# Black-Phoenix/CUDA-SfM

Measured on AMD Instinct MI355X. Metric: RANSAC E-matrix hypotheses/sec (8-point, fused scoring), inlier-mask parity vs CPU oracle, higher is better.
Workload: dtype f32

## Files before the change

### cuda-sfm_amd/csrc/common.hpp

```cpp
#pragma once
#include <hip/hip_runtime.h>
#include <stdint.h>
#include <stddef.h>
#include <string>
#include <atomic>
#include <type_traits>
#include "../../include/sfm_amd.h"
#include "pair_state.hpp"
#include "job_order.hpp"
#if SFM_AB
#include "../../include/sfm_amd_ab.h"
#endif

#if SFM_AB
#define SFM_SW(p, i) ((p).reserved[i])
#else
#define SFM_SW(p, i) 0
#endif

namespace sfm {

void set_error(const char *fmt, ...);

#define SFM_HIP_TRY(expr)                                                                      \
// ... 221 lines not shown
    hipEvent_t cells_ev = nullptr;
    hipStream_t cells_stream = nullptr;
    uint32_t cells_cap = 0, cells_mask = 0, cells_epoch = 0;
    uint32_t cand_h0 = 0, cand_seed = 0;
    const int32_t *cand_indices = nullptr;
    int cand_sweeps = 0;
    bool cand_given = false;
    hipStream_t pipe_stream = nullptr;
    hipEvent_t pipe_final[2] = { nullptr, nullptr }, pipe_call = nullptr;
    uint64_t *pipe_keys = nullptr;
    unsigned long long pipe_step = 0;
    bool pipe_pending = false;
    bool holds_ctx_ref = false;
    sfm::PairState state;
    float h_Kinv[9] = {};
    int pose_mode = SFM_POSE_REFERENCE;
    float *d_rstate = nullptr;
    float *d_rpoints = nullptr;
    float *d_rreproj = nullptr;
    void *d_rwork = nullptr;
    float *d_vstate = nullptr;
    float *d_vreproj = nullptr;
    void *d_vwork = nullptr;
    void *d_vhyp = nullptr;
    int *d_vcounts = nullptr;
    size_t cap_vhyps = 0;
    uint32_t view_hyps = 0;
    void *d_awork = nullptr;
    void *d_lwork = nullptr;
    void *d_lhyp = nullptr;
    size_t cap_lhyps = 0;
    int last_kernel = 0, last_grid = 0, last_block = 0, last_lds = 0;
};

namespace sfm {

int match_db_rows(const sfm_ctx *ctx, int n2);
int match_records(sfm_ctx *ctx, sfm_sift_point *d_sift1, int n1, const sfm_sift_point *d_sift2, int n2, int *out_idx);
int pose_chain(sfm_pair *pair, int mode, float *d_record);

int lane_contexts(sfm_ctx *ctx, int n, sfm_ctx **out);
int start_lanes_after(sfm_ctx *ctx, sfm_ctx *const *lanes, int n, hipEvent_t event);

int launch_ransac_score(sfm_pair *pair, ShardSlot &slot, hipStream_t stream, const sfm_ransac_params &p, uint32_t h0, uint32_t count,
                        unsigned long long *key2 = nullptr, const float *d_E_given = nullptr, bool serial = true);
int launch_ransac_finalize(sfm_pair *pair, const sfm_ransac_params &p, const unsigned long long *d_key, uint32_t hyp_host, bool from_key,
                           hipStream_t stream = nullptr, bool rederive = false);
int launch_permutation_indices(sfm_ctx *ctx, int n, uint32_t seed, int32_t *d_indices);
bool prefilter_usable(const sfm_pair *pair, const sfm_ransac_params &p, uint32_t count);
int prefilter_pick_rule(sfm_pair *pair, const sfm_ransac_params &p, uint32_t count);
int launch_score_prefilter(sfm_pair *pair, ShardSlot &slot, hipStream_t stream, const sfm_ransac_params &p, uint32_t h0, uint32_t count, unsigned long long *key2);
bool prefilter_sums_counts(const sfm_pair *pair, const sfm_ransac_params &p, uint32_t count);
int launch_pf_prep(sfm_pair *pair, ShardSlot &slot, hipStream_t stream, const sfm_ransac_params &p, uint32_t count);
int prefilter_tile_points(const sfm_pair *pair, const sfm_ransac_params &p);
int launch_pf_cells(sfm_pair *pair, hipStream_t stream, bool want_sorted = false, int tile = 0);
#if SFM_AB
int launch_score_prefilter_r2(sfm_pair *pair, ShardSlot &slot, hipStream_t stream, const sfm_ransac_params &p, uint32_t h0, uint32_t count, unsigned long long *key2);
int launch_score_mfma(sfm_pair *pair, ShardSlot &slot, hipStream_t stream, const sfm_ransac_params &p, uint32_t h0, uint32_t count);
int launch_prefilter_probe(sfm_ctx *ctx, const float *d_E, float thr, float B, const float pt[4], int survive_all, float *d_out);
int launch_prefilter_band_probe(sfm_ctx *ctx, const float *d_E, float thr, float B, const float box[8], int b_safe, const float pt[4], int survive_all, float *d_out);
#endif
int launch_ransac_fused(sfm_pair *pair, ShardSlot &slot, hipStream_t stream, const sfm_ransac_params &p, uint32_t h0, uint32_t count);
int launch_finalize_block(sfm_pair *pair, const sfm_ransac_params &p, const unsigned long long *d_key, uint32_t hyp_host, bool from_key,
                          hipStream_t stream, bool rederive);

int launch_fill_xu(sfm_pair *pair, const sfm_sift_point *d_data);
int launch_set_points(sfm_pair *pair, const float *d_X0, const float *d_X1);
int launch_pose_candidates(sfm_pair *pair, int mode);
int launch_choose_pose(sfm_pair *pair, int mode);
int launch_triangulate(sfm_pair *pair, int mode);
int launch_points_to_vbo(sfm_pair *pair, float *d_positions, float *d_velocities, float scale);
int launch_pair_record(sfm_pair *pair, int mode, float *d_record);
int launch_pose_chain(sfm_pair *pair, float *d_record);

int launch_refine(sfm_pair *pair, const sfm_refine_params &p);
int launch_refine_pairs(sfm_ctx *ctx, sfm_pair *const *pairs, int num_pairs, const sfm_refine_params &p, const uint8_t *const *d_masks);
size_t refine_work_bytes(int cap_points);
int refine_state_words();
int refine_pose_offset();
int refine_report_offset();

int launch_register(sfm_pair *pair, const sfm_sift_point *d_sift, const sfm_register_params &p, const float *d_points, const uint8_t *d_valid);
int launch_register_views(sfm_ctx *ctx, sfm_pair *const *pairs, int num_pairs, const sfm_sift_point *const *d_sifts, const sfm_register_params &p,
                          const float *const *d_points, const uint8_t *const *d_valid);
size_t register_work_bytes(int cap_points);
size_t register_hyp_bytes(size_t num_hypotheses);
int register_state_words();
int register_pose_offset();
int register_report_offset();

struct ViewPointsInputs { const sfm_sift_point *sift; const float *points; const uint8_t *valid; const float *pose2, *pose3; int pose_rows; };
int launch_view_points(sfm_pair *pair, const ViewPointsInputs &in, const sfm_view_points_params &p, const sfm_view_points_out &out);
int launch_view_points_views(sfm_ctx *ctx, sfm_pair *const *pairs, int num_pairs, const ViewPointsInputs *in, const sfm_view_points_params &p,
                             const sfm_view_points_out *outs);

struct AdjustInputs { const sfm_sift_point *sift; const float *points; const uint8_t *flags, *used2; const float *pose2, *pose3; int pose_rows; };
int launch_adjust(sfm_pair *pair, const AdjustInputs &in, const sfm_adjust_params &p, const sfm_adjust_out &out);
int launch_adjust_views(sfm_ctx *ctx, sfm_pair *const *pairs, int num_pairs, const AdjustInputs *in, const sfm_adjust_params &p, const sfm_adjust_out *outs);
size_t adjust_work_bytes(int cap_points);

struct AlignInputs { const float *points_a; const uint8_t *valid_a; const float *points_b; const uint8_t *valid_b; const int32_t *index; };
int launch_align(sfm_pair *a, sfm_pair *b, const AlignInputs &in, const sfm_align_params &p, const sfm_align_out &out);
int launch_align_pairs(sfm_ctx *ctx, sfm_pair *const *as, sfm_pair *const *bs, int num_links, const AlignInputs *in, const sfm_align_params &p,
                       const sfm_align_out *outs);
int launch_align_index(sfm_ctx *ctx, const sfm_sift_point *d_sift, int n, float min_score, float max_ambiguity, int32_t *d_index);
size_t align_work_bytes(int cap_points);
// ... 57 lines not shown
```

### cuda-sfm_amd/csrc/prefilter_lds.hpp

```cpp
#pragma once
#include "prefilter_record.hpp"

namespace sfm {

constexpr int kPfTileMax = 1024;
constexpr int kPfWaves = 16;
constexpr int kPfRing = 128;

constexpr int kPfERow = 10;
constexpr int kPfPassRows = 32, kPfPairRows = 64;
constexpr int pf_wave_bytes(int rows) { return rows * kPfERow * 4 + rows * 4; }
template <int RULE> struct PfLds {
    static constexpr int kFragsPerBlock = RULE == kPfRuleG ? 3 : 2;
    static constexpr int kBlockBytes = kFragsPerBlock * 64 * 16;
    static constexpr int kFrag = 0;
    static constexpr int kTileMax = kPfTileMax;
    int staged, pts, ring, wave, next, lut, bytes;
    __host__ __device__ explicit PfLds(int tile, int ring_entries = kPfRing, int entry_bytes = 8, int rows = RULE == kPfRuleG ? kPfPassRows : kPfPairRows)
    {
        staged = (tile + 63) & ~63;
        pts = kFrag + (staged / 32) * kBlockBytes;
        ring = pts + staged * 16;
        ring = (ring + ring_entries * entry_bytes - 1) & ~(ring_entries * entry_bytes - 1);
        wave = ring + kPfWaves * ring_entries * entry_bytes;
        next = wave + kPfWaves * pf_wave_bytes(rows);
        lut = next + 16;
        bytes = lut + kPfRingLutBytes;
    }
};
static_assert(kPfRing * 8 == 1024, "ring slots are addressed with (offset & 1023) | base");

static inline int pf_tile_points(int ld, int tmax)
{
    const int ntiles = (ld + tmax - 1) / tmax;
    const int t = ((ld + ntiles - 1) / ntiles + 31) & ~31;
    return t < 32 ? 32 : t;
}

constexpr unsigned long long kPfSumCountsMin = 1ull << 21;
static inline bool pf_sums_counts_at(unsigned count, int ld, int tile)
{
    return (unsigned long long)count * (unsigned long long)((ld + tile - 1) / tile) >= kPfSumCountsMin;
}

constexpr unsigned long long kPfPairPassesMin = 1ull << 22;
static inline bool pf_pairs_passes_at(unsigned count, int ld, int tile)
{
    return (unsigned long long)count * (unsigned long long)((ld + tile - 1) / tile) >= kPfPairPassesMin;
}

}
```

### cuda-sfm_amd/csrc/ransac.hip

```cpp
#include "ransac_device.hpp"
#include "block_ops.hpp"
#include "prefilter_record.hpp"

namespace sfm {

__device__ __forceinline__ void reset_keys(unsigned long long *key, unsigned long long *key2)
{
    if (blockIdx.x == 0 && threadIdx.x == 0) {
        key[0] = 0ull; key[1] = 0ull;
        if (key2) *key2 = 0ull;
    }
}

template <int WPE>
__global__ __launch_bounds__(64, WPE)
void ransac_solve_lanes(const float *__restrict__ X0, const float *__restrict__ X1, int ld, int n,
                        const int32_t *__restrict__ indices, uint32_t seed, uint32_t h0, uint32_t count,
                        int sweeps, float *__restrict__ Ecand, unsigned long long *zero_key, unsigned long long *zero_key2,
                        int *__restrict__ zero_counts, uint32_t *__restrict__ zero_ticks, uint32_t nzero)
{
    reset_keys(zero_key, zero_key2);
    const uint32_t i = blockIdx.x * blockDim.x + threadIdx.x;
    if (zero_ticks) for (uint32_t w = i; w < nzero; w += gridDim.x * blockDim.x) zero_ticks[w] = 0u;
    if (i >= count) return;
// ... 288 lines not shown
    sfm_ctx *ctx = pair->ctx;
    const uint32_t fused_max = p.jacobi_sweeps > 0 ? 4096u : 1024u;
    int kernel = p.kernel == SFM_KERNEL_AUTO ? (count <= fused_max ? SFM_KERNEL_FUSED : SFM_KERNEL_SPLIT) : p.kernel;
    if (d_E_given && kernel == SFM_KERNEL_FUSED) kernel = SFM_KERNEL_SPLIT;
    const bool self_clearing = !d_E_given && count > 0 && (kernel == SFM_KERNEL_SPLIT || kernel == SFM_KERNEL_PREFILTER);
    if (!self_clearing) {
        if (!pair->state.key_clean) SFM_HIP_TRY(hipMemsetAsync(s.key, 0, 2 * sizeof(unsigned long long), stream));
        if (key2) SFM_HIP_TRY(hipMemsetAsync(key2, 0, sizeof(unsigned long long), stream));
    }
    pair->state.key_clean = false;
    pair->state.last_count = serial ? count : 0;
    pair->cand_given = serial && d_E_given != nullptr;
    if (serial) { pair->cand_h0 = h0; pair->cand_seed = p.seed; pair->cand_indices = p.d_indices; pair->cand_sweeps = p.jacobi_sweeps; }
    if (count == 0) return SFM_OK;
    int rc = ensure_hyp_capacity(s, stream, count);
    if (rc != SFM_OK) return rc;

#if SFM_AB
    if (kernel == SFM_KERNEL_MFMA && pair->n >= 65536) kernel = SFM_KERNEL_SPLIT;
#endif
    if (kernel == SFM_KERNEL_PREFILTER && !prefilter_usable(pair, p, 0x40000000u)) kernel = SFM_KERNEL_SPLIT;
    if (p.kernel == SFM_KERNEL_AUTO && kernel == SFM_KERNEL_SPLIT && prefilter_usable(pair, p, count) && SFM_SW(p, 3) != 1) kernel = SFM_KERNEL_PREFILTER;
    pair->last_kernel = kernel;
    if (kernel == SFM_KERNEL_FUSED) {
        rc = launch_ransac_fused(pair, s, stream, p, h0, count);
        if (rc == SFM_OK && key2) SFM_HIP_TRY(hipMemcpyAsync(key2, s.key, sizeof(unsigned long long), hipMemcpyDeviceToDevice, stream));
        return rc;
    }

    const int tile = pair->ld < kTileMax ? pair->ld : kTileMax;
    const int ntiles = (pair->ld + tile - 1) / tile;
    int wpb = 16;
    while (wpb > 4 && (count + wpb - 1) / wpb < (uint32_t)ctx->num_cus) wpb >>= 1;
    const int nh = (wpb == 16 && count >= 8192u) ? 2 : 1;
    const uint32_t nbatch = (count + wpb * nh - 1) / (wpb * nh);
    const bool grid2d = ntiles > 1 && kernel == SFM_KERNEL_SPLIT && wpb == 16 && SFM_SW(p, 1) != 1;
    const bool prefilter = kernel == SFM_KERNEL_PREFILTER;

    const bool timed = ctx->timing && ctx->tcount < sfm_ctx::kTimingSlots;
    hipEvent_t *tev = timed ? ctx->tev[ctx->tcount] : nullptr;
    if (timed) SFM_HIP_TRY(hipEventRecord(tev[0], stream));
    const bool pf_tickets = prefilter && (SFM_SW(p, 3) == 2 || SFM_SW(p, 3) == 17);
    const bool pf_r2 = prefilter && SFM_SW(p, 3) == 2;
    PfScales pf_sc = {};
    if (prefilter) (void)prefilter_scales(p.threshold, pf_sc);
    if (prefilter && !pf_r2) {
        const int pf_rule = prefilter_pick_rule(pair, p, count);
        const int rcc = launch_pf_cells(pair, stream, pf_rule == kPfRuleBandTile, prefilter_tile_points(pair, p));
        if (rcc != SFM_OK) return rcc;
    }
    const bool pf_sums = prefilter && !pf_r2 && !pf_tickets && prefilter_sums_counts(pair, p, count);
    int *zero_counts = (grid2d || pf_tickets || pf_sums) ? s.counts : nullptr;
    const float4 *pts4 = (pair->state.have_pts4 && SFM_SW(p, 0) != 4) ? pair->d_pts4 : nullptr;
    const uint32_t nzero = (!prefilter || pf_sums) ? 0u : (pf_tickets ? (count + (uint32_t)kPfGroup - 1u) / (uint32_t)kPfGroup : 2u * count);
    uint32_t *zero_ticks = (prefilter && !pf_sums) ? s.tick : nullptr;
    if (zero_ticks && d_E_given) {
        SFM_HIP_TRY(hipMemsetAsync(s.tick, 0, (size_t)nzero * sizeof(uint32_t), stream));
        zero_ticks = nullptr;
    }
    bool need_prep = prefilter && !pf_r2;
    if (d_E_given) {
        SFM_HIP_TRY(hipMemcpyAsync(s.Ecand, d_E_given, (size_t)count * 9 * sizeof(float), hipMemcpyDeviceToDevice, stream));
        if (zero_counts) SFM_HIP_TRY(hipMemsetAsync(s.counts, 0, (size_t)count * sizeof(int), stream));
    }
#if SFM_AB
    else if (p.reserved[0] == 1 || p.reserved[0] == 7) {
        auto kern = p.reserved[0] == 1 ? ransac_solve_lanes<1> : ransac_solve_lanes<3>;
        hipLaunchKernelGGL(kern, dim3((count + 63) / 64), dim3(64), 0, stream,
                           pair->d_X[0], pair->d_X[1], pair->ld, pair->n, p.d_indices, p.seed, h0, count,
                           p.jacobi_sweeps, s.Ecand, s.key, key2, zero_counts, zero_ticks, nzero);
    }
#endif
    else if (p.jacobi_sweeps <= 0 && (SFM_SW(p, 0) == 3 || (SFM_SW(p, 0) == 0 && (pts4 != nullptr || count <= kScalarSolveMax)))) {
        const bool fuse = need_prep && SFM_SW(p, 3) != 3;
        const bool tile_rec = !fuse || pair->pf_rule == kPfRuleBandTile;
        hipLaunchKernelGGL(tile_rec ? ransac_solve_lanes1_qr : ransac_solve_lanes1_qr_rec, dim3((count + 63) / 64), dim3(64), 0, stream,
                           pair->d_X[0], pair->d_X[1], pair->ld, pair->n, p.d_indices, p.seed, h0, count,
                           p.jacobi_sweeps, s.Ecand, s.key, key2, zero_counts, zero_ticks, nzero, pts4,
                           fuse ? reinterpret_cast<PfRecord *>(s.pf) : nullptr, p.threshold, pf_sc, pair->d_bound, pair->d_cells, pair->cells_mask,
                           pair->pf_rule);
        if (fuse) need_prep = false;
    }
    else if (p.jacobi_sweeps <= 0)
        hipLaunchKernelGGL(ransac_solve_lanes2<true>, dim3((count + 127) / 128), dim3(64), 0, stream,
                           pair->d_X[0], pair->d_X[1], pair->ld, pair->n, p.d_indices, p.seed, h0, count,
                           p.jacobi_sweeps, s.Ecand, s.key, key2, zero_counts, zero_ticks, nzero, pts4);
#if SFM_AB
    else if (p.reserved[0] == 2)
        hipLaunchKernelGGL(ransac_solve_lanes2<false>, dim3((count + 127) / 128), dim3(64), 0, stream,
                           pair->d_X[0], pair->d_X[1], pair->ld, pair->n, p.d_indices, p.seed, h0, count,
                           p.jacobi_sweeps, s.Ecand, s.key, key2, zero_counts, zero_ticks, nzero, pts4);
#endif
    else
        hipLaunchKernelGGL(ransac_solve_lanes<2>, dim3((count + 63) / 64), dim3(64), 0, stream,
                           pair->d_X[0], pair->d_X[1], pair->ld, pair->n, p.d_indices, p.seed, h0, count,
                           p.jacobi_sweeps, s.Ecand, s.key, key2, zero_counts, zero_ticks, nzero);
    SFM_HIP_TRY(hipGetLastError());
    if (need_prep) {
        const int rcp = launch_pf_prep(pair, s, stream, p, count);
        if (rcp != SFM_OK) return rcp;
    }
    if (timed) SFM_HIP_TRY(hipEventRecord(tev[1], stream));

    const bool uz = pair->state.unit_z;
    const size_t lds = (uz ? (size_t)2 * kUnitZSecond : (size_t)6 * tile * sizeof(float)) + 16 * sizeof(unsigned long long);
    int per_cu = (int)((160 * 1024) / lds);
    if (per_cu > 2048 / (wpb * 64)) per_cu = 2048 / (wpb * 64);
    if (per_cu < 1) per_cu = 1;
    const uint32_t resident = (uint32_t)ctx->num_cus * (uint32_t)per_cu;
    const uint32_t min_batches = SFM_SW(p, 2) > 0 ? (uint32_t)SFM_SW(p, 2) : 8u;
    uint32_t blocks = nbatch / min_batches;
    if (blocks > 16u * (uint32_t)ctx->num_cus) blocks = 16u * (uint32_t)ctx->num_cus;
    if (blocks < resident) blocks = resident;
    int grid = (int)(nbatch < blocks ? nbatch : blocks);
    if (grid2d) {
        grid = (int)((blocks + ntiles - 1) / ntiles);
        if ((uint32_t)grid > nbatch) grid = (int)nbatch;
    }
    if (prefilter) {
#if SFM_AB
        if (pf_r2) rc = launch_score_prefilter_r2(pair, s, stream, p, h0, count, key2);
        else
#endif
        rc = launch_score_prefilter(pair, s, stream, p, h0, count, key2);
        if (rc == SFM_OK && pf_sums) rc = launch_argmax_counts(s, stream, h0, count, key2);
    }
#if SFM_AB
    else if (kernel == SFM_KERNEL_MFMA) {
        rc = launch_score_mfma(pair, s, stream, p, h0, count);
        if (rc == SFM_OK && key2) SFM_HIP_TRY(hipMemcpyAsync(key2, s.key, sizeof(unsigned long long), hipMemcpyDeviceToDevice, stream));
    }
#endif
    else if (grid2d) {
        rc = uz ? (nh == 2 ? launch_score_t<16, true, 2, true>(pair, s, stream, h0, count, p.threshold, tile, ntiles, grid, lds, key2)
                           : launch_score_t<16, true, 1, true>(pair, s, stream, h0, count, p.threshold, tile, ntiles, grid, lds, key2))
                : (nh == 2 ? launch_score_t<16, false, 2, true>(pair, s, stream, h0, count, p.threshold, tile, ntiles, grid, lds, key2)
                           : launch_score_t<16, false, 1, true>(pair, s, stream, h0, count, p.threshold, tile, ntiles, grid, lds, key2));
    }
    else if (uz) switch (wpb) {
    case 16: rc = nh == 2 ? launch_score_t<16, true, 2>(pair, s, stream, h0, count, p.threshold, tile, ntiles, grid, lds, key2)
                          : launch_score_t<16, true>(pair, s, stream, h0, count, p.threshold, tile, ntiles, grid, lds, key2); break;
    case 8:  rc = launch_score_t<8, true>(pair, s, stream, h0, count, p.threshold, tile, ntiles, grid, lds, key2); break;
    default: rc = launch_score_t<4, true>(pair, s, stream, h0, count, p.threshold, tile, ntiles, grid, lds, key2); break;
    }
    else switch (wpb) {
    case 16: rc = nh == 2 ? launch_score_t<16, false, 2>(pair, s, stream, h0, count, p.threshold, tile, ntiles, grid, lds, key2)
                          : launch_score_t<16, false>(pair, s, stream, h0, count, p.threshold, tile, ntiles, grid, lds, key2); break;
    case 8:  rc = launch_score_t<8, false>(pair, s, stream, h0, count, p.threshold, tile, ntiles, grid, lds, key2); break;
    default: rc = launch_score_t<4, false>(pair, s, stream, h0, count, p.threshold, tile, ntiles, grid, lds, key2); break;
    }
    if (rc == SFM_OK && timed) {
        SFM_HIP_TRY(hipEventRecord(tev[2], stream));
        ctx->tcount++;
    }
    return rc;
}

int launch_ransac_finalize(sfm_pair *pair, const sfm_ransac_params &p, const unsigned long long *d_key,
                           uint32_t hyp_host, bool from_key, hipStream_t stream, bool rederive)
{
    sfm_ctx *ctx = pair->ctx;
    if (!stream) stream = ctx->stream;
    (void)ctx;
    if (pair->cand_given && !rederive) {
        set_error("finalize after sfm_ransac_score_candidates: the candidates were supplied by the caller, not derived from 8-tuples");
        return SFM_E_STATE;
    }
    return launch_finalize_block(pair, p, d_key, hyp_host, from_key, stream, rederive);
}

int launch_permutation_indices(sfm_ctx *ctx, int n, uint32_t seed, int32_t *d_indices)
{
    const int h = n / 8;
    if (h == 0) return SFM_OK;
    int32_t *perm = new int32_t[n];
    for (int i = 0; i < n; ++i) perm[i] = i;
    const uint32_t base = hash32(hash32(seed) ^ 0x51F15EEDu);
    for (int i = n - 1; i > 0; --i) {
// ... 12 lines not shown
```

### cuda-sfm_amd/csrc/ransac_prefilter.hip

```cpp
#include "ransac_device.hpp"
#include "block_ops.hpp"
#include "prefilter_math.hpp"
#include "prefilter_record.hpp"
#include "prefilter_lds.hpp"

namespace sfm {

typedef float f16v __attribute__((ext_vector_type(16)));


__device__ constexpr int kPfESlot[9] = { 2, 6, 1, 3, 5, 7, 0, 4, 8 };
__device__ __forceinline__ uint32_t shift_in_reject(uint32_t rejected, float nt, float G)
{
    return __builtin_amdgcn_alignbit(rejected, __float_as_uint(fmaf(-nt, nt, G)), 31);
}

__device__ __forceinline__ uint32_t scan16(const f16v &nt, const f16v &G)
{
    uint32_t rejected = 0u;
#pragma unroll
    for (int r = 0; r < 16; ++r) rejected = shift_in_reject(rejected, nt[r], G[r]);
    return rejected;
}

// ... 38 lines not shown
    const v2f ab1 = __builtin_elementwise_fma(e44, yv, __builtin_elementwise_fma(e31, xu, p2));
    const float a2 = fmaf(p2.y, yv.x, fmaf(p0.y, xu.x, e8));
    const float nn = fmaf(yv.y, ab1.x, fmaf(xu.y, ab0.x, a2));
    const float n2 = nn * nn;
    const v2f dd = __builtin_elementwise_fma(ab1, ab1, ab0 * ab0);
    const float da = dd.x, db = dd.y;
    const float m = n2 * (da + db);
    const float tp = (da * db) * band.thr;
    const uint32_t mb = __float_as_uint(m), tb = __float_as_uint(tp);
    const uint32_t gap = __usad(mb, tb, 0u);
    const bool undecided = (gap < kBandUlps) || (tb < band.lo_bits) || (tb > band.hi_bits);
    bool in = m < tp;
    if (undecided) {
        const float t1 = (da == 0.0f) ? 0.0f : n2 / da;
        const float t2 = (db == 0.0f) ? 0.0f : n2 / db;
        in = (t1 + t2) < band.thr;
    }
    return in;
}

template <int RULE>
__device__ __forceinline__ PfFrags load_point_frags(lds_ch8 *frag_lane, int pb)
{
    lds_ch8 *p = frag_lane + pb * (PfLds<RULE>::kBlockBytes / 16);
    if (RULE != kPfRuleG) return PfFrags{ p[0], p[64], h8{} };
    return PfFrags{ p[0], p[64], p[128] };
}

template <int RULE>
__device__ __forceinline__ void mfma_step(const PfFrags &a, const PfFrags &b, f16v &G, f16v &nt)
{
    const f16v z = {};
    nt = __builtin_amdgcn_mfma_f32_32x32x16_f16(a.n0, b.n0, z, 0, 0, 0);
    if (RULE == kPfRuleG) G = __builtin_amdgcn_mfma_f32_32x32x16_f16(a.t, b.t, z, 0, 0, 0);
    nt = __builtin_amdgcn_mfma_f32_32x32x16_f16(a.n1, b.n1, nt, 0, 0, 0);
}

#define PF_SCHED_STEP()                                                 \
    do {                                                                \
        if (RULE != kPfRuleG) {                                         \
            __builtin_amdgcn_sched_group_barrier(0x008, 1, 0);          \
            __builtin_amdgcn_sched_group_barrier(0x002, 8, 0);          \
            __builtin_amdgcn_sched_group_barrier(0x008, 1, 0);          \
            __builtin_amdgcn_sched_group_barrier(0x002, 8, 0);          \
        } else {                                                        \
            __builtin_amdgcn_sched_group_barrier(0x008, 1, 0);          \
            __builtin_amdgcn_sched_group_barrier(0x002, 11, 0);         \
            __builtin_amdgcn_sched_group_barrier(0x008, 1, 0);          \
            __builtin_amdgcn_sched_group_barrier(0x002, 11, 0);         \
            __builtin_amdgcn_sched_group_barrier(0x008, 1, 0);          \
            __builtin_amdgcn_sched_group_barrier(0x002, 11, 0);         \
        }                                                               \
    } while (0)

constexpr int kPfVarTickets = 1;
constexpr int kPfVarDrainLocal = 2;
constexpr int kPfVarClosedDecode = 4;
constexpr int kPfVarAnswerEpilogue = 8;
constexpr int kPfVarDrainK1 = 16, kPfVarDrainK7 = 32;
constexpr int kPfVarSinglePass = 64;
constexpr int kPfVarPairDrain = 128;

constexpr int pf_score_waves_per_simd(int var, int rule, int fl2, int pipe, int wide, int prio)
{
    if ((var == 0 || var == kPfVarPairDrain) && rule == kPfRuleBandTile && !fl2 && !pipe && !wide && !prio) return 4;
    return ((var & kPfVarTickets) == 0 && (rule == kPfRuleBandTile || rule == kPfRuleBandPack) && !fl2 && !pipe && !wide && !prio) ? 5 : 4;
}

template <int W, int VAR = 0, int RULE = kPfRuleBandTile, int FL2 = 0, int PIPE = 0, int WIDE = 0, int PRIO = 0>
__global__ __launch_bounds__(W * 64, pf_score_waves_per_simd(VAR, RULE, FL2, PIPE, WIDE, PRIO))
void ransac_score_prefilter(const float *__restrict__ X0, const float *__restrict__ X1, int ld, int n,
                            const float *__restrict__ Ecand, const PfRecord *__restrict__ recs, uint32_t h0, uint32_t count, float thr,
                            int dynamic, int tile,
                            int *__restrict__ counts, uint32_t *__restrict__ tick,
                            unsigned long long *best_key, unsigned long long *best_key2, unsigned long long *__restrict__ clk,
                            const unsigned long long *__restrict__ bound_word, const uint32_t *__restrict__ tile_boxes)
{
    extern __shared__ __attribute__((aligned(16))) unsigned char smem[];
    const int lane = threadIdx.x & 63;
    const int wave = __builtin_amdgcn_readfirstlane(threadIdx.x >> 6);
    const bool probe = clk && blockIdx.x == 0 && blockIdx.y == 0 && threadIdx.x == 0;
    unsigned long long c0 = 0, w0 = 0;
    if (clk && blockIdx.x == 0 && blockIdx.y == 0 && wave == 0) { c0 = clock64(); w0 = wall_clock64(); }
#if SFM_AB
    const uint32_t trace_blk = blockIdx.y * gridDim.x + blockIdx.x;
    unsigned long long *trace = (clk && trace_blk < (uint32_t)kTraceBlocks) ? clk + 8 + (size_t)trace_blk * kTraceWords : nullptr;
    if (trace && threadIdx.x == 0) {
        trace[0] = wall_clock64();
        trace[2] = ((unsigned long long)__builtin_amdgcn_s_getreg((20 << 0) | (0 << 6) | (31 << 11)) << 32) |
                   (unsigned long long)__builtin_amdgcn_s_getreg((4 << 0) | (0 << 6) | (31 << 11));
        trace[3] = ((unsigned long long)blockIdx.y << 32) | blockIdx.x;
    }
#define PF_PHASE(k) do { if (probe1) clk[k] = wall_clock64() - w0; } while (0)
#else
#define PF_PHASE(k) do { } while (0)
#endif
    const int half = lane >> 5, row = lane & 31;
    uint32_t npass = (count + (uint32_t)kPfGroup - 1u) / (uint32_t)kPfGroup;
    const uint32_t nstatic = gridDim.x * (uint32_t)W;
    using LT = PfLds<RULE>;
    constexpr bool kBand = RULE != kPfRuleG, kTile = RULE == kPfRuleBandTile, kPack = RULE == kPfRuleBandPack || kTile;
    static_assert(!(FL2 && kPack) && !((VAR & kPfVarTickets) && kPack), "the recorded variants were built on the v_alignbit scan");
    constexpr bool kTail9 = kPack && W == 16 && !FL2 && !PIPE && !WIDE && !PRIO && !(VAR & kPfVarTickets);
    static_assert(kTail9 || (VAR & ~kPfVarTickets) == 0, "the pass-tail switches belong to the product's two rules");
    static_assert(!(VAR & kPfVarSinglePass) || (kTile && VAR == kPfVarSinglePass), "single passes: the per-tile rule's summing instance");
    static_assert(!(VAR & kPfVarPairDrain) || (kTile && VAR == kPfVarPairDrain), "paired passes drained between the scans: the per-tile rule's summing instance");
// ... 2 lines not shown
    constexpr int kRows = kPair ? kPfPairRows : kPfPassRows, kUnit = kRows;
    constexpr int kDrainMore = !kTail9 ? 0 : (VAR & kPfVarDrainK1) ? 1 : (VAR & kPfVarDrainK7) ? 7 : (VAR & kPfVarDrainLocal) ? 3 : 0;
    constexpr bool kDecodeTable = !(kTail9 && (VAR & kPfVarClosedDecode));
    constexpr bool kSumCounts = kTail9 && !(VAR & kPfVarAnswerEpilogue);
    constexpr int kRing = FL2 ? 256 : kPfRing;
    constexpr int kEnt = WIDE ? 16 : 8;
    static_assert(!WIDE || (kPack && !PIPE && !FL2), "wide entries: the packed scan's plain loop only");
    if (kPair) npass = (npass + 1u) >> 1;
    const LT L(tile, kRing, kEnt, kRows);
    float *etab = reinterpret_cast<float *>(smem + L.wave + wave * pf_wave_bytes(kRows));
    int *cnt = reinterpret_cast<int *>(etab + kRows * kPfERow);

    PfFrags afrag = {};
    h8 bfrag_n0 = {}, bfrag_n1 = {};
    uint32_t key0 = 0u;
    float rec_dn = 0.0f, rec_lin = 0.0f;
    float e_row[9] = {};
    auto fetch_pass = [&](uint32_t pass, PfFrags &af, uint32_t &k0, float (&e)[9], float &dn, float &lin) {
        const uint32_t hf = pass * (uint32_t)kUnit;
        const uint32_t h = hf + (uint32_t)min(kPair ? lane : row, (int)min((uint32_t)kUnit, count - hf) - 1);
        if (kTile) {
            const float *src = Ecand + 9 * (size_t)h;
#pragma unroll
            for (int k = 0; k < 9; ++k) e[k] = src[k];
            const uint4 rec = reinterpret_cast<const uint4 *>(recs)[h];
            k0 = rec.x; dn = __uint_as_float(rec.y); lin = __uint_as_float(rec.z);
            return;
        }
        const uint4 *r = reinterpret_cast<const uint4 *>(recs + h) + 2 * half;
        const uint4 r0 = r[0], r1 = r[1];
        if (kBand) pf_band_record_expand(r0, r1, half, af.n0, af.n1, k0);
        else pf_record_expand(r0, r1, half, af.n0, af.n1, af.t, k0);
        if (half == 0) {
            const float *src = Ecand + 9 * (size_t)h;
#pragma unroll
            for (int k = 0; k < 9; ++k) e[k] = src[k];
        }
    };
    auto install_rows = [&](const float (&e)[9]) {
        if (kPair || half == 0) {
            const int r = kPair ? lane : row;
#pragma unroll
            for (int k = 0; k < 9; ++k) etab[kRows * k + r] = e[kPfESlot[k]];
            cnt[r] = 0;
        }
    };
    uint32_t ps = blockIdx.x * (uint32_t)W + (uint32_t)wave;
    bool have = ps < npass;
    if (have) { fetch_pass(ps, afrag, key0, e_row, rec_dn, rec_lin); install_rows(e_row); }

    SFM_PHASE("stage_tile");
    uint32_t *next_idx = reinterpret_cast<uint32_t *>(smem + L.next);
    if (threadIdx.x == 0) *next_idx = (uint32_t)W;
    if constexpr (kCarry) {
        if (threadIdx.x < kPfRingLutBytes) smem[L.lut + threadIdx.x] = (unsigned char)pf_ring_lut_entry(threadIdx.x);
    } else
    if (kPack && kDecodeTable && threadIdx.x < 32) smem[L.lut + threadIdx.x] = (unsigned char)pf_pack_code((int)threadIdx.x);
    float pf_B = 0.0f;
    uint32_t bw[8] = {};
    uint32_t bw_lane = 0u;
    if (kTile) {
        pf_B = __uint_as_float((uint32_t)(__hip_atomic_load(reinterpret_cast<const uint32_t *>(bound_word), __ATOMIC_RELAXED, __HIP_MEMORY_SCOPE_AGENT)));
        bw_lane = __hip_atomic_load(tile_boxes + 8 * blockIdx.y + (lane & 7), __ATOMIC_RELAXED, __HIP_MEMORY_SCOPE_AGENT);
    }
    __syncthreads();
    const int tile_first = blockIdx.y * tile;
    for (int t = threadIdx.x; t < L.staged; t += W * 64) {
        const int p = tile_first + t;
        float u = 0.f, v = 0.f, x = 0.f, y = 0.f;
        const bool real = p < n && t < tile;
        if (kTile) {
            if (real) {
                const float4 q4 = reinterpret_cast<const float4 *>(X0)[p];
                u = q4.x; v = q4.y; x = q4.z; y = q4.w;
            }
        } else
        if (real) { u = X0[p]; v = X0[(size_t)ld + p]; x = X1[p]; y = X1[(size_t)ld + p]; }
        _Float16 bn[kPfSlots], bt[kPfSlotsT];
        prefilter_point_slots(u, v, x, y, real, bn, bt);
        reinterpret_cast<float4 *>(smem + L.pts)[t] = real ? make_float4(x, u, y, v) : make_float4(NAN, NAN, NAN, NAN);
        const int pb = t >> 5, col = t & 31;
        unsigned char *blk = smem + LT::kFrag + pb * LT::kBlockBytes;
#pragma unroll
        for (int ks = 0; ks < 2; ++ks)
#pragma unroll
            for (int hh = 0; hh < 2; ++hh) {
                h8 c;
#pragma unroll
                for (int j = 0; j < 8; ++j) c[j] = bn[ks * 16 + hh * 8 + j];
                *reinterpret_cast<h8 *>(blk + ks * 1024 + (hh * 32 + col) * 16) = c;
            }
        if (RULE == kPfRuleG) {
#pragma unroll
            for (int hh = 0; hh < 2; ++hh) {
                h8 c;
#pragma unroll
                for (int j = 0; j < 8; ++j) c[j] = bt[hh * 8 + j];
                *reinterpret_cast<h8 *>(blk + 2048 + (hh * 32 + col) * 16) = c;
            }
        }
    }
    __syncthreads();
    PfBox tbox = {};
    auto build_operands = [&](const float (&e)[9], uint32_t fl, float dn, float lin) {
        int half_l = half;
        float thr_l = thr, B_l = pf_B;
// ... 378 lines not shown
            k = wave_max(k);
            if (lane == 0 && k) {
                atomicMax(best_key, k);
                if (best_key2) atomicMax(best_key2, k);
            }
        }
        } else if (kSumCounts) {
        if (lane < nvalid_unit) {
            const int c = cnt[lane];
            if (c) __hip_atomic_fetch_add(&counts[h_first + lane], c, __ATOMIC_RELAXED, __HIP_MEMORY_SCOPE_AGENT);
        }
        if (have_next) {
            if (kTile) build_operands(e_next, key0n, dn_next, lin_next);
            else { afrag = afrag_next; key0 = key0n; }
            install_rows(e_next);
        }
        } else {
        uint32_t c_mine = 0u;
        unsigned long long old = 0ull;
        if (lane < nvalid) {
            c_mine = (uint32_t)cnt[lane];
            unsigned long long *acc = reinterpret_cast<unsigned long long *>(tick) + (h_first + (uint32_t)lane);
            old = atomicAdd(acc, (1ull << 32) | (unsigned long long)c_mine);
        }
        const int nvalid_done = nvalid;
        const uint32_t h_done = h_first;
        if (have_next) {
            if (kTile) build_operands(e_next, key0n, dn_next, lin_next);
            else { afrag = afrag_next; key0 = key0n; }
            install_rows(e_next);
        }
        unsigned long long k = 0;
        if (lane < nvalid_done && (uint32_t)(old >> 32) == gridDim.y - 1u) {
            const uint32_t total = (uint32_t)old + c_mine;
            counts[h_done + lane] = (int)total;
            k = pack_key(total, h0 + h_done + (uint32_t)lane);
        }
        if (__ballot(k != 0ull) != 0ull) {
            k = wave_max(k);
            if (lane == 0 && k > __hip_atomic_load(best_key, __ATOMIC_RELAXED, __HIP_MEMORY_SCOPE_AGENT)) {
                atomicMax(best_key, k);
                if (best_key2) atomicMax(best_key2, k);
            }
        }
        }
        PF_PHASE(5);
        ++passes_done;
        have = have_next;
        if (have_next) {
            ps = ps_next;
            if (VAR & kPfVarTickets) { afrag = afrag_next; key0 = key0n; install_rows(e_next); }
        }
    }
    SFM_PHASE("kernel_end");
    if (probe) { clk[6] = passes_done; clk[0] = clock64() - c0; clk[1] = wall_clock64() - w0; }
#if SFM_AB
    if (probe) clk[6] |= (unsigned long long)carried << 32;
    if (trace && lane == 0) {
        const unsigned long long tend = wall_clock64();
        trace[4 + wave] = tend;
        if (wave == 0) trace[1] = tend;
    }
#endif
}

constexpr int kPfBuckets = 1024 + 2;
constexpr int kPfBucketBlock = 256;

__device__ __forceinline__ int pf_bucket_of(const float4 q, float B)
{
    const float big = fmaxf(fmaxf(fabsf(q.x), fabsf(q.y)), fmaxf(fabsf(q.z), fabsf(q.w)));
    if (!(big <= 48.0f) || q.x != q.x || q.y != q.y || q.z != q.z || q.w != q.w) return kPfBuckets - 2;
    return (int)(pf_morton_key(q.x, q.y, -B, B, -B, B) >> 20);
}

__global__ __launch_bounds__(1024)
void pf_bucket_scan_kernel(uint32_t *__restrict__ hist, int nblocks, uint32_t *__restrict__ base, uint32_t *__restrict__ boxes, int nbox_words)
{
    for (int k = threadIdx.x; k < nbox_words; k += blockDim.x) boxes[k] = pf_order_bits(-INFINITY);
    __shared__ uint32_t total[kPfBuckets + 1024];
    for (int b = threadIdx.x; b < kPfBuckets; b += blockDim.x) {
        uint32_t run = 0u;
        for (int k = 0; k < nblocks; ++k) {
            const uint32_t c = hist[(size_t)k * kPfBuckets + b];
            hist[(size_t)k * kPfBuckets + b] = run;
            run += c;
        }
        total[b] = run;
    }
    __syncthreads();
    __shared__ uint32_t wsum[17];
    base[threadIdx.x] = block_scan<16>(total[threadIdx.x], wsum);
    if (threadIdx.x == 0) { base[1024] = wsum[16]; base[1025] = wsum[16] + total[1024]; }
}
static_assert(kPfBuckets == 1026, "pf_bucket_scan_kernel: 1024 Morton buckets scanned by 1024 threads + two special ones");

constexpr int kPfBoxTilesLds = 512;
__global__ __launch_bounds__(kPfBucketBlock)
void pf_bucket_scatter_kernel(const float4 *__restrict__ pts4, int n, int ld, const unsigned long long *__restrict__ bound_word,
                              const uint32_t *__restrict__ hist, const uint32_t *__restrict__ base, float4 *__restrict__ out,
                              int tile, int ntiles, uint32_t *__restrict__ boxes)
{
    constexpr int kWaves = kPfBucketBlock / 64;
    __shared__ unsigned short hw[kWaves][kPfBuckets];
    extern __shared__ uint32_t bx[];
    const int nlds = min(ntiles, kPfBoxTilesLds);
// ... 308 lines not shown
}

int launch_prefilter_probe(sfm_ctx *ctx, const float *d_E, float thr, float B, const float pt[4], int survive_all, float *d_out)
{
    PfScales sc;
    if (!prefilter_scales(thr, sc)) { set_error("threshold %g outside the pre-filter's range", (double)thr); return SFM_E_INVALID; }
    hipLaunchKernelGGL(pf_probe_kernel, dim3(1), dim3(64), 0, ctx->stream, d_E, thr, B, sc, pt[0], pt[1], pt[2], pt[3], survive_all,
                       reinterpret_cast<PfRecord *>(d_out + 128), d_out);
    SFM_HIP_TRY(hipGetLastError());
    return SFM_OK;
}
#endif

static int pf_rule_switch(const sfm_ransac_params &p)
{
    if (SFM_SW(p, 3) == 4 || SFM_SW(p, 3) >= 16) return kPfRuleG;
    if (SFM_SW(p, 3) == 5 || SFM_SW(p, 1) == 5 || SFM_SW(p, 1) == 7 || SFM_SW(p, 1) == 9) return kPfRuleBand;
    if (SFM_SW(p, 3) == 6 || SFM_SW(p, 1) == 11 || SFM_SW(p, 1) == 12) return kPfRuleBandPack;
    if (SFM_SW(p, 3) == 7 || SFM_SW(p, 1) == 13 || SFM_SW(p, 1) == 14 || SFM_SW(p, 1) == 15) return kPfRuleBandTile;
    return -1;
}

constexpr uint64_t kPfOrderFirstCallPairs = 1ull << 33;
int prefilter_pick_rule(sfm_pair *pair, const sfm_ransac_params &p, uint32_t count)
{
    int rule = pf_rule_switch(p);
    if (rule < 0) {
        const bool ordered = pair->sorted_epoch == pair->bound_epoch && pair->d_pts4s != nullptr;
        const bool first = pair->pf_seen_epoch != pair->bound_epoch;
        rule = (!ordered && first && (uint64_t)count * (uint64_t)pair->ld < kPfOrderFirstCallPairs) ? kPfRuleBandPack : kPfRuleBandTile;
    }
    pair->pf_seen_epoch = pair->bound_epoch;
    pair->pf_rule = rule;
    return rule;
}

bool prefilter_usable(const sfm_pair *pair, const sfm_ransac_params &p, uint32_t count)
{
    PfScales sc;
    return pair->state.unit_z && pair->state.have_bound && count >= 16384u && (uint64_t)count * (uint64_t)pair->ld >= (1ull << 27) && prefilter_scales(p.threshold, sc);
}

static int pf_tile_of(const sfm_pair *pair, const sfm_ransac_params &p)
{
    if (SFM_SW(p, 1) == 7 && pair->pf_rule == kPfRuleBand) return pf_tile_points(pair->ld, 1536);
    return pf_tile_points(pair->ld, kPfTileMax);
}

int prefilter_tile_points(const sfm_pair *pair, const sfm_ransac_params &p) { return pf_tile_of(pair, p); }

static int pf_tail_var(const sfm_pair *pair, const sfm_ransac_params &p, uint32_t count)
{
    const bool large = pf_sums_counts_at(count, pair->ld, pf_tile_of(pair, p));
    if (SFM_SW(p, 1) == 19) return 0;
    if (SFM_SW(p, 1) == 20) return pair->pf_rule == kPfRuleBandTile ? kPfVarSinglePass : 0;
    if (SFM_SW(p, 1) == 21) return pair->pf_rule == kPfRuleBandTile ? kPfVarPairDrain : 0;
    if (pair->pf_rule == kPfRuleBandTile && SFM_SW(p, 1) == 16) return kPfVarDrainK1;
    if (pair->pf_rule == kPfRuleBandTile && SFM_SW(p, 1) == 17) return kPfVarDrainK7;
    int var = 0;
    const bool lab = SFM_SW(p, 3) >= 8 && SFM_SW(p, 3) < 16;
    if (lab && (SFM_SW(p, 3) & 1)) var |= kPfVarDrainLocal;
    if (lab && (SFM_SW(p, 3) & 2)) var |= kPfVarClosedDecode;
    const bool sum = (lab && (SFM_SW(p, 3) & 4)) ? false : (large || (SFM_SW(p, 1) >= 16 && SFM_SW(p, 1) <= 18));
    if (!sum) var |= kPfVarAnswerEpilogue;
    if (var == 0 && pair->pf_rule == kPfRuleBandTile && !pf_pairs_passes_at(count, pair->ld, pf_tile_of(pair, p))) var = kPfVarSinglePass;
    return var;
}

bool prefilter_sums_counts(const sfm_pair *pair, const sfm_ransac_params &p, uint32_t count)
{
    const bool product_rule = pair->pf_rule == kPfRuleBandTile || pair->pf_rule == kPfRuleBandPack;
    const bool variant = SFM_SW(p, 1) == 5 || (SFM_SW(p, 1) >= 11 && SFM_SW(p, 1) <= 15);
    return product_rule && !variant && !(pf_tail_var(pair, p, count) & kPfVarAnswerEpilogue);
}

int launch_score_prefilter(sfm_pair *pair, ShardSlot &s, hipStream_t stream, const sfm_ransac_params &p, uint32_t h0, uint32_t count, unsigned long long *key2)
{
    sfm_ctx *ctx = pair->ctx;
    PfScales sc;
    if (!prefilter_scales(p.threshold, sc)) { set_error("threshold %g outside the pre-filter's range", (double)p.threshold); return SFM_E_INVALID; }
    const int waves = (SFM_SW(p, 1) == 5 || SFM_SW(p, 1) == 12) ? 12 : kPfWaves;
    const int tile = pf_tile_of(pair, p);
    const int ntiles = (pair->ld + tile - 1) / tile;
    const uint32_t npass = (count + (uint32_t)kPfGroup - 1u) / (uint32_t)kPfGroup;
    const int rule = pair->pf_rule;
    const int tail_var = pf_tail_var(pair, p, count);
    const bool wide = rule == kPfRuleBandTile && SFM_SW(p, 1) == 13;
    const bool paired_units = rule == kPfRuleBandTile && (tail_var == 0 || tail_var == kPfVarPairDrain) && waves == kPfWaves && !wide && SFM_SW(p, 1) != 14 && SFM_SW(p, 1) != 15;
    const uint32_t nunits = paired_units ? (npass + 1u) / 2u : npass;
    const uint32_t iters = (nunits + (uint32_t)waves - 1) / (uint32_t)waves;
    uint32_t cols = (uint32_t)ctx->num_cus / (uint32_t)ntiles;
    if (SFM_SW(p, 2) > 0) cols = (uint32_t)SFM_SW(p, 2);
    if (cols > iters) cols = iters;
    if (cols < 1) cols = 1;
    const int dynamic = SFM_SW(p, 1) == 2 ? 0 : 1;
    const int var = SFM_SW(p, 3) >= 16 ? SFM_SW(p, 3) - 16 : 0;
    const bool fl2 = rule == kPfRuleBand && waves == kPfWaves && SFM_SW(p, 1) == 9;
    const int lds_bytes = wide ? PfLds<kPfRuleBand>(tile, kPfRing, 16, kPfPassRows).bytes : fl2 ? PfLds<kPfRuleBand>(tile, 256, 8, kPfPassRows).bytes
                        : rule != kPfRuleG ? PfLds<kPfRuleBand>(tile, kPfRing, 8, paired_units ? kPfPairRows : kPfPassRows).bytes : PfLds<kPfRuleG>(tile).bytes;
    if (lds_bytes > 160 * 1024) { set_error("pre-filter tile of %d points needs %d bytes of LDS", tile, lds_bytes); return SFM_E_INVALID; }
    auto launch = [&](auto kernel) -> int {
        const int rc_lds = allow_big_lds(ctx, reinterpret_cast<const void *>(kernel));
        if (rc_lds != SFM_OK) return rc_lds;
        const float *x0 = rule == kPfRuleBandTile ? reinterpret_cast<const float *>(pair->d_pts4s) : pair->d_X[0];
        hipLaunchKernelGGL(kernel, dim3(cols, ntiles), dim3(waves * 64), lds_bytes, stream,
                           x0, pair->d_X[1], pair->ld, pair->n, s.Ecand, reinterpret_cast<const PfRecord *>(s.pf), h0, count, p.threshold,
                           dynamic, tile, s.counts, s.tick, s.key, key2, pair->d_clk, pair->d_bound, pair->d_tile_boxes);
        return SFM_OK;
    };
    int rcl;
#if SFM_AB
    if (rule == kPfRuleG && waves == 12) rcl = launch(&ransac_score_prefilter<12, 0, kPfRuleG>);
    else if (rule == kPfRuleG && var == 1) rcl = launch(&ransac_score_prefilter<16, 1, kPfRuleG>);
    else if (rule == kPfRuleG) rcl = launch(&ransac_score_prefilter<16, 0, kPfRuleG>);
    else if (waves == 12) rcl = launch(&ransac_score_prefilter<12, 0, kPfRuleBand>);
    else if (fl2) rcl = launch(&ransac_score_prefilter<16, 0, kPfRuleBand, 1>);
    else if (rule == kPfRuleBand) rcl = launch(&ransac_score_prefilter<16, 0, kPfRuleBand>);
    else if (SFM_SW(p, 1) == 11) rcl = launch(&ransac_score_prefilter<16, 0, kPfRuleBandPack, 0, 1>);
    else if (SFM_SW(p, 1) == 12) rcl = launch(&ransac_score_prefilter<12, 0, kPfRuleBandPack, 0, 1>);
    else if (wide) rcl = launch(&ransac_score_prefilter<16, 0, kPfRuleBandTile, 0, 0, 1>);
    else if (rule == kPfRuleBandTile && SFM_SW(p, 1) == 14) rcl = launch(&ransac_score_prefilter<16, 0, kPfRuleBandTile, 0, 0, 0, 1>);
    else if (rule == kPfRuleBandTile && SFM_SW(p, 1) == 15) rcl = launch(&ransac_score_prefilter<16, 0, kPfRuleBandTile, 0, 0, 0, 2>);
    else if (tail_var != 0 && tail_var != kPfVarAnswerEpilogue && tail_var != kPfVarSinglePass) {
        rcl = SFM_E_INVALID;
#define PF_TAIL_CASE(V) case V: rcl = rule == kPfRuleBandPack ? launch(&ransac_score_prefilter<16, V, kPfRuleBandPack>) : launch(&ransac_score_prefilter<16, V, kPfRuleBandTile>); break
        switch (tail_var) {
        PF_TAIL_CASE(2); PF_TAIL_CASE(4); PF_TAIL_CASE(6); PF_TAIL_CASE(10); PF_TAIL_CASE(12); PF_TAIL_CASE(14);
        case kPfVarDrainK1: rcl = launch(&ransac_score_prefilter<16, kPfVarDrainK1, kPfRuleBandTile>); break;
        case kPfVarDrainK7: rcl = launch(&ransac_score_prefilter<16, kPfVarDrainK7, kPfRuleBandTile>); break;
        case kPfVarPairDrain: rcl = launch(&ransac_score_prefilter<16, kPfVarPairDrain, kPfRuleBandTile>); break;
        default: set_error("pass-tail switches %d: no such instance", tail_var); break;
        }
#undef PF_TAIL_CASE
    }
    else
#endif
    if (tail_var & kPfVarAnswerEpilogue) rcl = rule == kPfRuleBandPack ? launch(&ransac_score_prefilter<16, kPfVarAnswerEpilogue, kPfRuleBandPack>)
                                                                       : launch(&ransac_score_prefilter<16, kPfVarAnswerEpilogue, kPfRuleBandTile>);
    else if (rule == kPfRuleBandPack) rcl = launch(&ransac_score_prefilter<16, 0, kPfRuleBandPack>);
    else if (tail_var == kPfVarSinglePass) rcl = launch(&ransac_score_prefilter<16, kPfVarSinglePass, kPfRuleBandTile>);
    else rcl = launch(&ransac_score_prefilter<16, 0, kPfRuleBandTile>);
    (void)var; (void)fl2; (void)wide; (void)tail_var;
    if (rcl != SFM_OK) return rcl;
    SFM_HIP_TRY(hipGetLastError());
    pair->last_grid = (int)cols * ntiles; pair->last_block = waves * 64; pair->last_lds = lds_bytes;
    return SFM_OK;
}

}
```

Before: 2.858 billion.

## Fuse argmax over summed counts into prefilter kernel via per-column tickets

In the sums-counts prefilter path, the separate argmax_counts launch is replaced by an in-kernel epilogue. Each block counts finished waves in LDS, and the last wave takes a per-column ticket in global memory. The last tile in each column then scans that column's hypothesis chunks with buffer loads and updates the best key atomically. This removes a kernel launch and a full re-read of the counts array, at the cost of ticket zeroing, atomics and a serialized tail scan done by one wave per column.

```diff
diff --git a/cuda-sfm_amd/csrc/common.hpp b/cuda-sfm_amd/csrc/common.hpp
--- a/cuda-sfm_amd/csrc/common.hpp
+++ b/cuda-sfm_amd/csrc/common.hpp
@@ -297,6 +297,7 @@
 int launch_score_prefilter(sfm_pair *pair, ShardSlot &slot, hipStream_t stream, const sfm_ransac_params &p, uint32_t h0, uint32_t count, unsigned long long *key2);
 bool prefilter_sums_counts(const sfm_pair *pair, const sfm_ransac_params &p, uint32_t count);
 int launch_pf_prep(sfm_pair *pair, ShardSlot &slot, hipStream_t stream, const sfm_ransac_params &p, uint32_t count);
+uint32_t prefilter_argmax_tickets(const sfm_pair *pair, const sfm_ransac_params &p, uint32_t count);
 int prefilter_tile_points(const sfm_pair *pair, const sfm_ransac_params &p);
 int launch_pf_cells(sfm_pair *pair, hipStream_t stream, bool want_sorted = false, int tile = 0);
 #if SFM_AB
diff --git a/cuda-sfm_amd/csrc/prefilter_lds.hpp b/cuda-sfm_amd/csrc/prefilter_lds.hpp
--- a/cuda-sfm_amd/csrc/prefilter_lds.hpp
+++ b/cuda-sfm_amd/csrc/prefilter_lds.hpp
@@ -43,6 +43,25 @@
     return (unsigned long long)count * (unsigned long long)((ld + tile - 1) / tile) >= kPfSumCountsMin;
 }
 
+__host__ __device__ inline uint32_t pf_unit_of(uint32_t got, uint32_t col, uint32_t grid_waves, uint32_t waves)
+{
+    return (got / waves) * grid_waves + col * waves + (got % waves);
+}
+__host__ __device__ inline uint32_t pf_column_of_hyp(uint32_t hyp, uint32_t chunk, uint32_t cols) { return (hyp / chunk) % cols; }
+__host__ __device__ inline uint32_t pf_column_chunks(uint32_t count, uint32_t chunk, uint32_t cols, uint32_t col)
+{
+    const uint32_t nchunks = (uint32_t)(((unsigned long long)count + chunk - 1u) / chunk);
+    return col < nchunks ? (nchunks - col - 1u) / cols + 1u : 0u;
+}
+__host__ __device__ inline uint32_t pf_column_chunk_first(uint32_t k, uint32_t chunk, uint32_t cols, uint32_t col) { return (col + k * cols) * chunk; }
+__host__ __device__ inline uint32_t pf_column_vec_first(uint32_t j, uint32_t chunk, uint32_t cols, uint32_t col)
+{
+    return pf_column_chunk_first(j / (chunk / 4u), chunk, cols, col) + (j % (chunk / 4u)) * 4u;
+}
+__host__ __device__ inline bool pf_vec_whole(uint32_t first, uint32_t count) { return count >= 4u && first <= count - 4u; }
+__host__ __device__ inline bool pf_ticket_closes(uint32_t drawn, uint32_t tiles) { return drawn == tiles - 1u; }
+constexpr unsigned kPfInKernelArgmaxMax = 1u << 29;
+
 constexpr unsigned long long kPfPairPassesMin = 1ull << 22;
 static inline bool pf_pairs_passes_at(unsigned count, int ld, int tile)
 {
diff --git a/cuda-sfm_amd/csrc/ransac.hip b/cuda-sfm_amd/csrc/ransac.hip
--- a/cuda-sfm_amd/csrc/ransac.hip
+++ b/cuda-sfm_amd/csrc/ransac.hip
@@ -364,8 +364,9 @@
     const bool pf_sums = prefilter && !pf_r2 && !pf_tickets && prefilter_sums_counts(pair, p, count);
     int *zero_counts = (grid2d || pf_tickets || pf_sums) ? s.counts : nullptr;
     const float4 *pts4 = (pair->state.have_pts4 && SFM_SW(p, 0) != 4) ? pair->d_pts4 : nullptr;
-    const uint32_t nzero = (!prefilter || pf_sums) ? 0u : (pf_tickets ? (count + (uint32_t)kPfGroup - 1u) / (uint32_t)kPfGroup : 2u * count);
-    uint32_t *zero_ticks = (prefilter && !pf_sums) ? s.tick : nullptr;
+    const uint32_t pf_col_tickets = pf_sums ? prefilter_argmax_tickets(pair, p, count) : 0u;
+    const uint32_t nzero = !prefilter ? 0u : pf_sums ? pf_col_tickets : (pf_tickets ? (count + (uint32_t)kPfGroup - 1u) / (uint32_t)kPfGroup : 2u * count);
+    uint32_t *zero_ticks = (prefilter && nzero != 0u) ? s.tick : nullptr;
     if (zero_ticks && d_E_given) {
         SFM_HIP_TRY(hipMemsetAsync(s.tick, 0, (size_t)nzero * sizeof(uint32_t), stream));
         zero_ticks = nullptr;
@@ -435,7 +436,7 @@
         else
 #endif
         rc = launch_score_prefilter(pair, s, stream, p, h0, count, key2);
-        if (rc == SFM_OK && pf_sums) rc = launch_argmax_counts(s, stream, h0, count, key2);
+        if (rc == SFM_OK && pf_sums && pf_col_tickets == 0u) rc = launch_argmax_counts(s, stream, h0, count, key2);
     }
 #if SFM_AB
     else if (kernel == SFM_KERNEL_MFMA) {
diff --git a/cuda-sfm_amd/csrc/ransac_prefilter.hip b/cuda-sfm_amd/csrc/ransac_prefilter.hip
--- a/cuda-sfm_amd/csrc/ransac_prefilter.hip
+++ b/cuda-sfm_amd/csrc/ransac_prefilter.hip
@@ -114,6 +114,43 @@
             __builtin_amdgcn_sched_group_barrier(0x002, 11, 0);         \
         }                                                               \
     } while (0)
+
+constexpr int kPfFoldLoads = 10;
+template <int CHUNK>
+__device__ __forceinline__ unsigned long long pf_column_key(const int *counts, uint32_t h0, uint32_t count, uint32_t col, uint32_t cols, int lane)
+{
+    constexpr uint32_t kVec = CHUNK / 4;
+    static_assert(CHUNK % 4 == 0 && (kVec & (kVec - 1u)) == 0u, "a chunk is a power of two of whole vectors");
+    const uint32_t nvec = pf_column_chunks(count, CHUNK, cols, col) * kVec;
+    const __amdgpu_buffer_rsrc_t rs = __builtin_amdgcn_make_buffer_rsrc(const_cast<int *>(counts), 0, (int)(count * 4u), 0x00027000);
+    unsigned long long best = 0ull;
+    for (uint32_t j0 = 0; j0 < nvec; j0 += 64u * kPfFoldLoads) {
+        u4v v[kPfFoldLoads];
+#pragma unroll
+        for (int u = 0; u < kPfFoldLoads; ++u)
+            v[u] = __builtin_amdgcn_raw_buffer_load_b128(rs, (int)(pf_column_vec_first(j0 + 64u * (uint32_t)u + (uint32_t)lane, CHUNK, cols, col) * 4u), 0, 16);
+        __builtin_amdgcn_sched_barrier(0);
+#pragma unroll
+        for (int u = 0; u < kPfFoldLoads; ++u) {
+            uint32_t j = j0 + 64u * (uint32_t)u + (uint32_t)lane;
+            asm volatile("" : "+v"(j));
+            const uint32_t first = pf_column_vec_first(j, CHUNK, cols, col);
+            const bool whole = j < nvec && pf_vec_whole(first, count);
+#pragma unroll
+            for (int c = 0; c < 4; ++c) {
+                const unsigned long long key = pack_key(v[u][c], h0 + first + (uint32_t)c);
+                best = (whole && key > best) ? key : best;
+            }
+        }
+    }
+    const uint32_t tail = count & ~3u;
+    if (pf_column_of_hyp(tail, CHUNK, cols) == col && tail + (uint32_t)lane < count) {
+        const int c = __hip_atomic_load(counts + tail + lane, __ATOMIC_RELAXED, __HIP_MEMORY_SCOPE_AGENT);
+        const unsigned long long key = pack_key((uint32_t)c, h0 + tail + (uint32_t)lane);
+        best = key > best ? key : best;
+    }
+    return wave_max(best);
+}
 
 constexpr int kPfVarTickets = 1;
 constexpr int kPfVarDrainLocal = 2;
@@ -222,6 +259,7 @@
     SFM_PHASE("stage_tile");
     uint32_t *next_idx = reinterpret_cast<uint32_t *>(smem + L.next);
     if (threadIdx.x == 0) *next_idx = (uint32_t)W;
+    if constexpr (kSumCounts) { if (threadIdx.x == 0) next_idx[1] = 0u; }
     if constexpr (kCarry) {
         if (threadIdx.x < kPfRingLutBytes) smem[L.lut + threadIdx.x] = (unsigned char)pf_ring_lut_entry(threadIdx.x);
     } else
@@ -706,6 +744,26 @@
             if (VAR & kPfVarTickets) { afrag = afrag_next; key0 = key0n; install_rows(e_next); }
         }
     }
+    if constexpr (kSumCounts) {
+        if (tick) {
+            asm volatile("s_waitcnt vmcnt(0)" ::: "memory");
+            uint32_t arrived = 0u;
+            if (lane == 0) arrived = __hip_atomic_fetch_add(next_idx + 1, 1u, __ATOMIC_RELAXED, __HIP_MEMORY_SCOPE_WORKGROUP);
+            arrived = (uint32_t)__builtin_amdgcn_readfirstlane((int)arrived);
+            if (arrived == (uint32_t)W - 1u) {
+                uint32_t t = 0u;
+                if (lane == 0) t = __hip_atomic_fetch_add(tick + blockIdx.x, 1u, __ATOMIC_RELAXED, __HIP_MEMORY_SCOPE_AGENT);
+                t = (uint32_t)__builtin_amdgcn_readfirstlane((int)t);
+                if (pf_ticket_closes(t, gridDim.y)) {
+                    const unsigned long long k = pf_column_key<W * kUnit>(counts, h0, count, blockIdx.x, gridDim.x, lane);
+                    if (lane == 0 && k) {
+                        atomicMax(best_key, k);
+                        if (best_key2) atomicMax(best_key2, k);
+                    }
+                }
+            }
+        }
+    }
     SFM_PHASE("kernel_end");
     if (probe) { clk[6] = passes_done; clk[0] = clock64() - c0; clk[1] = wall_clock64() - w0; }
 #if SFM_AB
@@ -1120,8 +1178,8 @@
 static int pf_tail_var(const sfm_pair *pair, const sfm_ransac_params &p, uint32_t count)
 {
     const bool large = pf_sums_counts_at(count, pair->ld, pf_tile_of(pair, p));
-    if (SFM_SW(p, 1) == 19) return 0;
-    if (SFM_SW(p, 1) == 20) return pair->pf_rule == kPfRuleBandTile ? kPfVarSinglePass : 0;
+    if (SFM_SW(p, 1) == 19 || SFM_SW(p, 1) == 23) return 0;
+    if (SFM_SW(p, 1) == 20 || SFM_SW(p, 1) == 24) return pair->pf_rule == kPfRuleBandTile ? kPfVarSinglePass : 0;
     if (SFM_SW(p, 1) == 21) return pair->pf_rule == kPfRuleBandTile ? kPfVarPairDrain : 0;
     if (pair->pf_rule == kPfRuleBandTile && SFM_SW(p, 1) == 16) return kPfVarDrainK1;
     if (pair->pf_rule == kPfRuleBandTile && SFM_SW(p, 1) == 17) return kPfVarDrainK7;
@@ -1142,25 +1200,44 @@
     return product_rule && !variant && !(pf_tail_var(pair, p, count) & kPfVarAnswerEpilogue);
 }
 
+struct PfShape { int waves, tile, ntiles, tail_var; bool wide, paired_units; uint32_t cols; };
+static PfShape pf_shape(const sfm_pair *pair, const sfm_ransac_params &p, uint32_t count)
+{
+    PfShape sh;
+    sh.waves = (SFM_SW(p, 1) == 5 || SFM_SW(p, 1) == 12) ? 12 : kPfWaves;
+    sh.tile = pf_tile_of(pair, p);
+    sh.ntiles = (pair->ld + sh.tile - 1) / sh.tile;
+    const uint32_t npass = (count + (uint32_t)kPfGroup - 1u) / (uint32_t)kPfGroup;
+    sh.tail_var = pf_tail_var(pair, p, count);
+    sh.wide = pair->pf_rule == kPfRuleBandTile && SFM_SW(p, 1) == 13;
+    sh.paired_units = pair->pf_rule == kPfRuleBandTile && (sh.tail_var == 0 || sh.tail_var == kPfVarPairDrain) && sh.waves == kPfWaves && !sh.wide && SFM_SW(p, 1) != 14 && SFM_SW(p, 1) != 15;
+    const uint32_t nunits = sh.paired_units ? (npass + 1u) / 2u : npass;
+    const uint32_t iters = (nunits + (uint32_t)sh.waves - 1) / (uint32_t)sh.waves;
+    sh.cols = (uint32_t)pair->ctx->num_cus / (uint32_t)sh.ntiles;
+    if (SFM_SW(p, 2) > 0) sh.cols = (uint32_t)SFM_SW(p, 2);
+    if (sh.cols > iters) sh.cols = iters;
+    if (sh.cols < 1) sh.cols = 1;
+    return sh;
+}
+
+uint32_t prefilter_argmax_tickets(const sfm_pair *pair, const sfm_ransac_params &p, uint32_t count)
+{
+    if (!prefilter_sums_counts(pair, p, count) || count > kPfInKernelArgmaxMax) return 0u;
+    if (SFM_SW(p, 1) >= 16 && SFM_SW(p, 1) <= 22) return 0u;
+    return pf_shape(pair, p, count).cols;
+}
+
 int launch_score_prefilter(sfm_pair *pair, ShardSlot &s, hipStream_t stream, const sfm_ransac_params &p, uint32_t h0, uint32_t count, unsigned long long *key2)
 {
     sfm_ctx *ctx = pair->ctx;
     PfScales sc;
     if (!prefilter_scales(p.threshold, sc)) { set_error("threshold %g outside the pre-filter's range", (double)p.threshold); return SFM_E_INVALID; }
-    const int waves = (SFM_SW(p, 1) == 5 || SFM_SW(p, 1) == 12) ? 12 : kPfWaves;
-    const int tile = pf_tile_of(pair, p);
-    const int ntiles = (pair->ld + tile - 1) / tile;
-    const uint32_t npass = (count + (uint32_t)kPfGroup - 1u) / (uint32_t)kPfGroup;
-    const int rule = pair->pf_rule;
-    const int tail_var = pf_tail_var(pair, p, count);
-    const bool wide = rule == kPfRuleBandTile && SFM_SW(p, 1) == 13;
-    const bool paired_units = rule == kPfRuleBandTile && (tail_var == 0 || tail_var == kPfVarPairDrain) && waves == kPfWaves && !wide && SFM_SW(p, 1) != 14 && SFM_SW(p, 1) != 15;
-    const uint32_t nunits = paired_units ? (npass + 1u) / 2u : npass;
-    const uint32_t iters = (nunits + (uint32_t)waves - 1) / (uint32_t)waves;
-    uint32_t cols = (uint32_t)ctx->num_cus / (uint32_t)ntiles;
-    if (SFM_SW(p, 2) > 0) cols = (uint32_t)SFM_SW(p, 2);
-    if (cols > iters) cols = iters;
-    if (cols < 1) cols = 1;
+    const PfShape sh = pf_shape(pair, p, count);
+    const int waves = sh.waves, tile = sh.tile, ntiles = sh.ntiles, rule = pair->pf_rule, tail_var = sh.tail_var;
+    const bool wide = sh.wide, paired_units = sh.paired_units;
+    const uint32_t cols = sh.cols;
+    const bool sums = prefilter_sums_counts(pair, p, count);
+    uint32_t *tick = (sums && prefilter_argmax_tickets(pair, p, count) == 0u) ? nullptr : s.tick;
     const int dynamic = SFM_SW(p, 1) == 2 ? 0 : 1;
     const int var = SFM_SW(p, 3) >= 16 ? SFM_SW(p, 3) - 16 : 0;
     const bool fl2 = rule == kPfRuleBand && waves == kPfWaves && SFM_SW(p, 1) == 9;
@@ -1173,7 +1250,7 @@
         const float *x0 = rule == kPfRuleBandTile ? reinterpret_cast<const float *>(pair->d_pts4s) : pair->d_X[0];
         hipLaunchKernelGGL(kernel, dim3(cols, ntiles), dim3(waves * 64), lds_bytes, stream,
                            x0, pair->d_X[1], pair->ld, pair->n, s.Ecand, reinterpret_cast<const PfRecord *>(s.pf), h0, count, p.threshold,
-                           dynamic, tile, s.counts, s.tick, s.key, key2, pair->d_clk, pair->d_bound, pair->d_tile_boxes);
+                           dynamic, tile, s.counts, tick, s.key, key2, pair->d_clk, pair->d_bound, pair->d_tile_boxes);
         return SFM_OK;
     };
     int rcl;
```

Result: no change. 2.857 billion (median of 2 runs) (-0.0%).
